# ml4ai/mliis

Hardware: AMD Instinct MI355X
Metric: inner-loop images/sec (EfficientLab-6-3, 224x224, 5-shot) (higher is better)
Workload: dtype f32 (the long-K decoder convs and their filter gradients with every operand split exactly into three bf16 terms on the matrix cores, 6 term products, f32 accumulate: fp32-equivalent products; everything else the fp32 instruction)

## Files before the change

### mliis_amd/csrc/conv_gemm_kernels.hpp

```cpp
#pragma once
#include <stdlib.h>

#include <type_traits>

#include "bn_fold.hpp"
#include "common.hpp"

namespace mliis {

typedef float f32x4 __attribute__((ext_vector_type(4)));

struct ConvGemmParams {
  const float* A;
  int lda;
  int Nimg, H, W;
  int C;
  int ntaps, dil, sign;
  const float* B;
  long long b_tap_stride;
  int ldb;
  int Nout;
  float* Cmat;
  int ldc;
  const float* bias;
// ... 826 lines not shown
            const float gq = (rok && cok) ? v * rscale : 0.f;
            const float xh = (side[r][j] - bmean[j]) * brstd[j];
            s1[j] += gq;
            s2[j] = fmaf(gq, xh, s2[j]);
          } else if constexpr (MODE == 1 || MODE == 2) {
            const float u0 = MODE == 2 ? swish_f(v) : v;
            const float u = rok ? u0 : 0.f;
            s1[j] += u;
            s2[j] = fmaf(u, u, s2[j]);
          }
        }
      }
    };
    if (bnb) epilogue(std::integral_constant<int, 3>{});
    else if (gated_part) epilogue(std::integral_constant<int, 4>{});
    else if (stats && p.stats_swish) epilogue(std::integral_constant<int, 2>{});
    else if (stats) epilogue(std::integral_constant<int, 1>{});
    else epilogue(std::integral_constant<int, 0>{});
    if (p.c_block != 0) {
      constexpr int QN = 4 * NT;
#pragma unroll
      for (int u = 0; u < NT; ++u) {
        const int e = lane + 64 * u;
        const int q4 = e >> 4, row = e & 15;
        const int m = rg * 16 + row, n = n0 + q4 * 4;
        const float4 v4 = ld4(&stage[wave][row * SROW + q4 * 4]);
        if (q4 < QN && m < M && n < p.Nout) {
          if (p.c_block == 4) {
            st4(p.Cmat + ((long long)(n >> 2) * M + m) * 4, v4);
          } else {
            float* d0 = p.Cmat + ((long long)(n >> 1) * M + m) * 2;
            *reinterpret_cast<float2*>(d0) = make_float2(v4.x, v4.y);
            *reinterpret_cast<float2*>(d0 + (long long)M * 2) = make_float2(v4.z, v4.w);
          }
        }
      }
    } else {
      constexpr int QN = 4 * NT;
#pragma unroll
      for (int u = 0; u < NT; ++u) {
        const int e = lane + 64 * u;
        const int row = e / QN, q4 = e - row * QN;
        const int m = rg * 16 + row, n = n0 + q4 * 4;
        const float4 v4 = ld4(&stage[wave][row * SROW + q4 * 4]);
        if (m < M && n < p.Nout) {
          if (PREC == 1 && p.out_bf16) stq(reinterpret_cast<bf16s*>(p.Cmat) + (long long)m * p.ldc + n, v4);
          else st4(p.Cmat + (long long)m * p.ldc + n, v4);
        }
      }
    }
    if (gated_part) {
#pragma unroll
      for (int j = 0; j < NT; ++j) {
        float a = gp0[j], b = gp1[j];
        a += __shfl_xor(a, 16, 64);
        b += __shfl_xor(b, 16, 64);
        a += __shfl_xor(a, 32, 64);
        b += __shfl_xor(b, 32, 64);
        const int n = n0 + j * 16 + l15;
        if (g == 0 && n < p.Nout) {
          p.gp_part[((long long)rg * 2 + 0) * p.Nout + n] = a;
          p.gp_part[((long long)rg * 2 + 1) * p.Nout + n] = b;
        }
      }
    }
    if constexpr (PF) {
#pragma unroll
      for (int kg = 0; kg < KC; ++kg) a_cur[kg] = a_nxt[kg];
      if constexpr (AIN) {
        if (rg + stride < row_groups) bn_in(rg + stride, a_cur, r_nxt, is_nxt);
      }
    } else {
      if (rg + stride < row_groups) {
        load_a(rg + stride, a_cur);
        load_side(rg + stride, r_cur, is_cur);
        bn_in(rg + stride, a_cur, r_cur, is_cur);
      }
    }
  }
  if (!stats) return;
#pragma unroll
  for (int j = 0; j < NT; ++j) {
    float a = s1[j], b = s2[j];
    a += __shfl_xor(a, 16, 64);
    b += __shfl_xor(b, 16, 64);
    a += __shfl_xor(a, 32, 64);
    b += __shfl_xor(b, 32, 64);
    if (g == 0) {
      red[wave][0][j * 16 + l15] = a;
      red[wave][1][j * 16 + l15] = b;
    }
  }
  __syncthreads();
  for (int idx = t; idx < 2 * 16 * NT; idx += 64 * kStreamWaves) {
    const int v = idx / (16 * NT), col = idx - v * (16 * NT);
    const int n = n0 + col;
    if (n < p.Nout) {
      float a = red[0][v][col];
#pragma unroll
      for (int wv = 1; wv < kStreamWaves; ++wv) a += red[wv][v][col];
      p.stats_part[((long long)blockIdx.x * 2 + v) * p.Nout + n] = a;
    }
  }
}

template <int KC, int NT, int WV, int PREC>
__global__ __launch_bounds__(64 * WV, (KC <= 6 && KC * NT <= 8) ? 4 : 2) void conv1x1_ksplit_k(ConvGemmParams p, int row_groups) {
  constexpr int BN = 16 * NT, RS = BN + 4, QN = BN / 4;
  __shared__ __attribute__((aligned(16))) float red[WV][16][RS];
  const int t = threadIdx.x, lane = t & 63, wave = t >> 6;
  const int l15 = lane & 15, g = lane >> 4;
  const int M = p.Nimg * p.H * p.W, HW = p.H * p.W;
  const int bx = blockIdx.x, by = blockIdx.y;
  const int n0 = by * BN;
  const int k0 = wave * 16 * KC;
  const __amdgpu_buffer_rsrc_t rA = __builtin_amdgcn_make_buffer_rsrc((void*)p.A, 0, kBufRecords, 0x00020000);
  const __amdgpu_buffer_rsrc_t rB = __builtin_amdgcn_make_buffer_rsrc((void*)p.B, 0, kBufRecords, 0x00020000);
  const __amdgpu_buffer_rsrc_t rS = __builtin_amdgcn_make_buffer_rsrc((void*)(p.a_scale ? p.a_scale : p.A), 0, kBufRecords, 0x00020000);
  const bool gated = p.a_scale != nullptr;
  float4 bv[KC][NT];
#pragma unroll
  for (int kg = 0; kg < KC; ++kg)
#pragma unroll
    for (int j = 0; j < NT; ++j) {
      const int n = n0 + j * 16 + l15, k = k0 + kg * 16 + g * 4;
      bv[kg][j] = buf_ld4(rB, (n < p.Nout && k < p.C) ? (unsigned)((n * p.ldb + k) * 4) : kOob);
    }
  constexpr int KC2 = (KC + 1) / 2;
  const float b_qscale = PREC == 2 ? fp8_weight_scale(p.b_amax) : 1.0f;
  const float out_scale = PREC == 2 ? 1.0f / (p.a_qscale * b_qscale) : 1.0f;
  bf16x8 bq16[PREC == 1 ? KC2 : 1][PREC == 1 ? NT : 1];
  long bq8[PREC == 2 ? KC2 : 1][PREC == 2 ? NT : 1];
  if constexpr (PREC != 0) {
#pragma unroll
    for (int k2 = 0; k2 < KC2; ++k2)
#pragma unroll
      for (int j = 0; j < NT; ++j) {
        const float4 lo = bv[2 * k2][j], hi = (2 * k2 + 1 < KC) ? bv[(2 * k2 + 1 < KC) ? 2 * k2 + 1 : 0][j] : f4zero();
        if constexpr (PREC == 1) bq16[k2][j] = pack_bf16x8(lo, hi);
        else bq8[k2][j] = pack_fp8x8(lo, hi, b_qscale);
      }
  }
  const bool fin = t < 16 * QN;
  const int frow = fin ? t / QN : 0, fq = fin ? t - frow * QN : 0;
  const int fn = n0 + fq * 4;
  const bool fcol = fin && fn < p.Nout;
  const float4 fbias = (fcol && p.bias != nullptr) ? ld4(p.bias + fn) : f4zero();
  float4 s1 = f4zero(), s2 = f4zero();
  const bool stats = p.stats_part != nullptr;
  const bool bnb = stats && p.bnb_x != nullptr;
  const float4 bmean = (bnb && fcol) ? ld4(p.bnb_mean + fn) : f4zero(), brstd = (bnb && fcol) ? ld4(p.bnb_rstd + fn) : f4zero();
  __shared__ __attribute__((aligned(16))) float sgate[2][16 * KC * WV];
  auto load_a = [&](int rg, float4* a) {
    const int m = rg * 16 + l15;
    const bool rok = rg < row_groups && m < M;
#pragma unroll
    for (int kg = 0; kg < KC; ++kg) {
      const int k = k0 + kg * 16 + g * 4;
      const bool ok = rok && k < p.C;
      if (PREC == 1 && p.a_bf16) a[kg] = buf_ld4_bf16(rA, ok ? (unsigned)((m * p.lda + k) * 2) : kOob);
      else a[kg] = buf_ld4(rA, ok ? (unsigned)((m * p.lda + k) * 4) : kOob);
    }
  };
  constexpr int GQ = 4 * KC * WV;
  auto gate_fetch = [&](int rg) {
    float4 v = f4zero();
    if (gated && t < 2 * GQ) {
      const int im = t / GQ, q = t - im * GQ;
      const int m0 = rg * 16;
      const int img = (m0 < M ? m0 : M - 1) / HW + im;
      if (rg < row_groups && img < p.Nimg && q * 4 < p.C) v = buf_ld4(rS, (unsigned)((img * p.C + q * 4) * 4));
    }
    return v;
  };
  auto gate_apply = [&](int rg, float4* a) {
    const int m = rg * 16 + l15;
    const int im = (m < M ? m : M - 1) / HW - (rg * 16 < M ? rg * 16 : M - 1) / HW;
#pragma unroll
    for (int kg = 0; kg < KC; ++kg) a[kg] = f4mul(a[kg], ld4(&sgate[im][k0 + kg * 16 + g * 4]));
  };
  int rg = bx;
  float4 a_cur[KC], a_nxt[KC];
  float4 gq = gate_fetch(rg);
  load_a(rg, a_cur);
  for (; rg < row_groups; rg += gridDim.x) {
    load_a(rg + gridDim.x, a_nxt);
    if (gated) {
      if (t < 2 * GQ) st4(&sgate[0][0] + t * 4, gq);
      __syncthreads();
      gate_apply(rg, a_cur);
      gq = gate_fetch(rg + gridDim.x);
    }
    float4 pre_dst = f4zero(), pre_x = f4zero();
    {
      const int mf = rg * 16 + frow;
      const bool pok = fcol && mf < M;
      if (p.accumulate && pok) pre_dst = ld4(p.Cmat + (long long)mf * p.ldc + fn);
      if (bnb && pok) pre_x = ld4(p.bnb_x + (long long)mf * p.bnb_ldx + fn);
    }
    f32x4 acc[NT];
#pragma unroll
    for (int j = 0; j < NT; ++j) acc[j] = (f32x4){0.f, 0.f, 0.f, 0.f};
    if constexpr (PREC == 0) {
#pragma unroll
      for (int kg = 0; kg < KC; ++kg)
#pragma unroll
        for (int sI = 0; sI < 4; ++sI) {
          const float a = sI == 0 ? a_cur[kg].x : sI == 1 ? a_cur[kg].y : sI == 2 ? a_cur[kg].z : a_cur[kg].w;
#pragma unroll
          for (int j = 0; j < NT; ++j) {
            const float b = sI == 0 ? bv[kg][j].x : sI == 1 ? bv[kg][j].y : sI == 2 ? bv[kg][j].z : bv[kg][j].w;
            acc[j] = __builtin_amdgcn_mfma_f32_16x16x4f32(a, b, acc[j], 0, 0, 0);
          }
        }
    } else {
#pragma unroll
      for (int k2 = 0; k2 < KC2; ++k2) {
        const float4 lo = a_cur[2 * k2], hi = (2 * k2 + 1 < KC) ? a_cur[(2 * k2 + 1 < KC) ? 2 * k2 + 1 : 0] : f4zero();
        if constexpr (PREC == 1) {
          const bf16x8 a8 = pack_bf16x8(lo, hi);
#pragma unroll
          for (int j = 0; j < NT; ++j) acc[j] = __builtin_amdgcn_mfma_f32_16x16x32_bf16(a8, bq16[k2][j], acc[j], 0, 0, 0);
        } else {
          const long a8 = pack_fp8x8(lo, hi, p.a_qscale);
#pragma unroll
          for (int j = 0; j < NT; ++j) acc[j] = __builtin_amdgcn_mfma_f32_16x16x32_fp8_fp8(a8, bq8[k2][j], acc[j], 0, 0, 0);
        }
      }
    }
#pragma unroll
    for (int r = 0; r < 4; ++r)
#pragma unroll
      for (int j = 0; j < NT; ++j) red[wave][g * 4 + r][j * 16 + l15] = PREC == 2 ? acc[j][r] * out_scale : acc[j][r];
    __syncthreads();
    const int m = rg * 16 + frow;
    if (fcol && m < M) {
      float4 v = ld4(&red[0][frow][fq * 4]);
#pragma unroll
      for (int w = 1; w < WV; ++w) v = f4add(v, ld4(&red[w][frow][fq * 4]));
      v = f4add(v, fbias);
      float* dst = p.Cmat + (long long)m * p.ldc + fn;
      if (p.accumulate) v = f4add(v, pre_dst);
      st4(dst, v);
      if (bnb) {
        const float4 xv = pre_x;
        if (p.bnb_scale != nullptr) v = f4scale(v, p.bnb_scale[m / HW]);
        const float4 xh = make_float4((xv.x - bmean.x) * brstd.x, (xv.y - bmean.y) * brstd.y, (xv.z - bmean.z) * brstd.z,
                                      (xv.w - bmean.w) * brstd.w);
        s1 = f4add(s1, v);
        s2 = f4fma(v, xh, s2);
      } else if (stats) {
        if (p.stats_swish) v = make_float4(swish_f(v.x), swish_f(v.y), swish_f(v.z), swish_f(v.w));
        s1 = f4add(s1, v);
        s2 = f4fma(v, v, s2);
      }
    }
    __syncthreads();
#pragma unroll
    for (int kg = 0; kg < KC; ++kg) a_cur[kg] = a_nxt[kg];
  }
  if (!stats) return;
  float4* fold = reinterpret_cast<float4*>(&red[0][0][0]);
  if (fin) {
    fold[(0 * 16 + frow) * QN + fq] = s1;
    fold[(1 * 16 + frow) * QN + fq] = s2;
  }
  __syncthreads();
  if (t < 2 * QN) {
    const int v = t / QN, q = t - v * QN;
    const int n = n0 + q * 4;
    if (n < p.Nout) {
      float4 a = fold[(v * 16) * QN + q];
#pragma unroll
      for (int r = 1; r < 16; ++r) a = f4add(a, fold[(v * 16 + r) * QN + q]);
      st4(p.stats_part + ((long long)bx * 2 + v) * p.Nout + n, a);
    }
  }
}

struct FilterGradParams {
  const float* X;
  int ldx;
  int Nimg, H, W;
  int C;
  int ntaps, dil;
  const float* dY;
  int lddy;
  int Nout;
  float* partial;
  int rows_per_split;
  const float* x_scale;
  int multitap;
  int x_bf16 = 0, dy_bf16 = 0;
};

template <int TMF, int NT>
struct FilterSm {
  static constexpr int BCI = 64 * TMF, BN = 16 * NT, BKM = 32;
  static constexpr int LDX = BCI + 16;
  static constexpr int LDD = (BN % 32 == 0) ? BN + 16 : BN;
  static constexpr int BUF_FLOATS = BKM * LDX + BKM * LDD;
};

template <int TMF, int NT, bool SC, bool BF>
__device__ __forceinline__ void conv_filter_grad2_body(const FilterGradParams& p, float* __restrict__ sm, int bx, int by, int bz) {
  constexpr int BCI = 64 * TMF, BN = 16 * NT, BKM = 32;
  constexpr int LDX = FilterSm<TMF, NT>::LDX;
  constexpr int LDD = FilterSm<TMF, NT>::LDD;
  constexpr int X_PER_THREAD = (BKM * (BCI / 4)) / 256;
  constexpr int D_TOTAL = BKM * (BN / 4);
  constexpr int D_PER_THREAD = (D_TOTAL + 255) / 256;
  constexpr int X_RSTEP = 256 / (BCI / 4);
  constexpr int BUF_FLOATS = FilterSm<TMF, NT>::BUF_FLOATS;
  constexpr int PF = (TMF == 2 && (SC || NT >= 8)) ? 1 : 2;

  const int t = threadIdx.x;
  const int lane = t & 63, wave = t >> 6;
  const int l15 = lane & 15, g = lane >> 4;
  const int M = p.Nimg * p.H * p.W;
  const bool mt = p.multitap != 0;
  const int cblocks = mt ? 1 : (p.C + BCI - 1) / BCI;
  const int tap = mt ? 0 : bx / cblocks;
  const int ci0 = mt ? 0 : (bx - tap * cblocks) * BCI;
  const int n0 = by * BN;
  const int mbeg = bz * p.rows_per_split;
  int mend = mbeg + p.rows_per_split;
  if (mend > M) mend = M;
  const int HW = p.H * p.W;
  const int adv_h = BKM / p.W, adv_w = BKM - adv_h * p.W;
  const bool xbf = BF && p.x_bf16 != 0, dbf = BF && p.dy_bf16 != 0;
  const int xb = xbf ? 2 : 4, db = dbf ? 2 : 4;

  const __amdgpu_buffer_rsrc_t rX = __builtin_amdgcn_make_buffer_rsrc((void*)p.X, 0, kBufRecords, 0x00020000);
  const __amdgpu_buffer_rsrc_t rD = __builtin_amdgcn_make_buffer_rsrc((void*)p.dY, 0, kBufRecords, 0x00020000);
  const __amdgpu_buffer_rsrc_t rS = __builtin_amdgcn_make_buffer_rsrc((void*)(SC ? p.x_scale : p.X), 0, kBufRecords, 0x00020000);

  const int x_cq = t % (BCI / 4);
  const int x_r0 = t / (BCI / 4);
  int l_tap = tap, l_c = ci0 + x_cq * 4;
  if (mt) {
    l_tap = (x_cq * 4) / p.C;
    l_c = x_cq * 4 - l_tap * p.C;
  }
  const bool x_cok = mt ? l_tap < p.ntaps : l_c < p.C;
  int dh = 0, dw = 0;
  if (p.ntaps > 1) {
    dh = (l_tap / 3 - 1) * p.dil;
    dw = (l_tap % 3 - 1) * p.dil;
  }
  int x_m[X_PER_THREAD], x_h[X_PER_THREAD], x_w[X_PER_THREAD], x_n[X_PER_THREAD];
  unsigned x_off[X_PER_THREAD];
#pragma unroll
  for (int i = 0; i < X_PER_THREAD; ++i) {
    const int m = mbeg + x_r0 + X_RSTEP * i;
    x_m[i] = m;
    x_n[i] = m / HW;
    const int rem = m - x_n[i] * HW;
    x_h[i] = rem / p.W;
    x_w[i] = rem - x_h[i] * p.W;
    x_off[i] = (unsigned)((((long long)m + (long long)dh * p.W + dw) * p.ldx + l_c) * xb);
  }
  const unsigned x_step = (unsigned)(BKM * p.ldx * xb);
  int d_m[D_PER_THREAD];
  unsigned d_off[D_PER_THREAD];
  bool d_ok[D_PER_THREAD];
#pragma unroll
  for (int i = 0; i < D_PER_THREAD; ++i) {
    const int idx = t + 256 * i;
    const int r = idx / (BN / 4), nq = idx - r * (BN / 4);
    d_m[i] = mbeg + r;
    d_ok[i] = (idx < D_TOTAL) && (n0 + nq * 4 < p.Nout);
    d_off[i] = (unsigned)((((long long)mbeg + r) * p.lddy + n0 + nq * 4) * db);
  }
  const unsigned d_step = (unsigned)(BKM * p.lddy * db);

  float4 rx[PF][X_PER_THREAD], rs[PF][X_PER_THREAD], rd[PF][D_PER_THREAD];
  auto load_chunk = [&](float4* rx_, float4* rs_, float4* rd_) {
#pragma unroll
    for (int i = 0; i < X_PER_THREAD; ++i) {
      const bool ok = x_cok & (x_m[i] < mend) & ((unsigned)(x_h[i] + dh) < (unsigned)p.H) & ((unsigned)(x_w[i] + dw) < (unsigned)p.W);
      if (BF && xbf) rx_[i] = buf_ld4_bf16(rX, ok ? x_off[i] : kOob);
      else rx_[i] = buf_ld4(rX, ok ? x_off[i] : kOob);
      if (SC) rs_[i] = buf_ld4(rS, ok ? (unsigned)((x_n[i] * p.C + l_c) * 4) : kOob);
      x_m[i] += BKM;
      x_off[i] += x_step;
      x_w[i] += adv_w;
      x_h[i] += adv_h;
      if (x_w[i] >= p.W) {
        x_w[i] -= p.W;
        ++x_h[i];
      }
      if (x_h[i] >= p.H) {
        const int k = x_h[i] / p.H;
        x_h[i] -= k * p.H;
        x_n[i] += k;
      }
    }
#pragma unroll
    for (int i = 0; i < D_PER_THREAD; ++i) {
      if (BF && dbf) rd_[i] = buf_ld4_bf16(rD, (d_ok[i] & (d_m[i] < mend)) ? d_off[i] : kOob);
      else rd_[i] = buf_ld4(rD, (d_ok[i] & (d_m[i] < mend)) ? d_off[i] : kOob);
      d_m[i] += BKM;
      d_off[i] += d_step;
    }
  };
  auto store_chunk = [&](float* buf, const float4* rx_, const float4* rs_, const float4* rd_) {
    float* smX = buf;
    float* smD = buf + BKM * LDX;
#pragma unroll
    for (int i = 0; i < X_PER_THREAD; ++i) {
      float4 v = rx_[i];
      if (SC) v = f4mul(v, rs_[i]);
      st4(smX + (x_r0 + X_RSTEP * i) * LDX + x_cq * 4, v);
    }
#pragma unroll
    for (int i = 0; i < D_PER_THREAD; ++i) {
      const int idx = t + 256 * i;
      if (idx < D_TOTAL) {
        const int r = idx / (BN / 4), nq = idx - r * (BN / 4);
        st4(smD + r * LDD + nq * 4, rd_[i]);
      }
    }
  };

  f32x4 acc[TMF][NT];
#pragma unroll
  for (int i = 0; i < TMF; ++i)
#pragma unroll
    for (int j = 0; j < NT; ++j) acc[i][j] = (f32x4){0.f, 0.f, 0.f, 0.f};

  load_chunk(rx[0], rs[0], rd[0]);
  store_chunk(sm, rx[0], rs[0], rd[0]);
  if (PF == 2) load_chunk(rx[PF - 1], rs[PF - 1], rd[PF - 1]);
  __syncthreads();
  int cur = 0;
  const bool wave_live = mt ? wave * TMF * 16 < p.ntaps * p.C : ci0 + wave * TMF * 16 < p.C;
  auto step = [&](auto UC) {
    constexpr int U = decltype(UC)::value;
    constexpr int NX = (U + 1) % PF;
    load_chunk(rx[U], rs[U], rd[U]);
    const float* smX = sm + cur * BUF_FLOATS;
    const float* smD = smX + BKM * LDX;
    if (!wave_live) {
    } else if constexpr (BF) {
      bf16x8 a8[TMF], b8[NT];
#pragma unroll
      for (int kk = 0; kk < BKM / 4; ++kk) {
        const int mrow = kk * 4 + g;
#pragma unroll
        for (int i = 0; i < TMF; ++i) a8[i][kk] = (__bf16)smX[mrow * LDX + (wave * TMF + i) * 16 + l15];
#pragma unroll
        for (int j = 0; j < NT; ++j) b8[j][kk] = (__bf16)smD[mrow * LDD + j * 16 + l15];
      }
#pragma unroll
      for (int i = 0; i < TMF; ++i)
#pragma unroll
        for (int j = 0; j < NT; ++j) acc[i][j] = __builtin_amdgcn_mfma_f32_16x16x32_bf16(a8[i], b8[j], acc[i][j], 0, 0, 0);
    } else
#pragma unroll
    for (int kk = 0; kk < BKM / 4; ++kk) {
      const int mrow = kk * 4 + g;
      float a[TMF], b[NT];
#pragma unroll
      for (int i = 0; i < TMF; ++i) a[i] = smX[mrow * LDX + (wave * TMF + i) * 16 + l15];
#pragma unroll
      for (int j = 0; j < NT; ++j) b[j] = smD[mrow * LDD + j * 16 + l15];
#pragma unroll
      for (int i = 0; i < TMF; ++i)
#pragma unroll
        for (int j = 0; j < NT; ++j) acc[i][j] = __builtin_amdgcn_mfma_f32_16x16x4f32(a[i], b[j], acc[i][j], 0, 0, 0);
    }
    store_chunk(sm + (cur ^ 1) * BUF_FLOATS, rx[NX], rs[NX], rd[NX]);
    cur ^= 1;
    __syncthreads();
  };
  typedef std::integral_constant<int, 0> U0;
  typedef std::integral_constant<int, 1 % PF> U1;
  const int nchunks = (mend - mbeg + BKM - 1) / BKM;
  int it = 0;
  for (; it + 4 <= nchunks; it += 4) {
    step(U0{});
    step(U1{});
    step(U0{});
    step(U1{});
  }
  if (it < nchunks) step(U0{});
  if (it + 1 < nchunks) step(U1{});
  if (it + 2 < nchunks) step(U0{});

  const long long Ktot = (long long)p.ntaps * p.C;
#pragma unroll
  for (int i = 0; i < TMF; ++i)
#pragma unroll
    for (int r = 0; r < 4; ++r) {
      const int ci = ci0 + (wave * TMF + i) * 16 + g * 4 + r;
      if (ci >= (mt ? p.ntaps * p.C : p.C)) continue;
#pragma unroll
      for (int j = 0; j < NT; ++j) {
        const int n = n0 + j * 16 + l15;
        if (n < p.Nout) p.partial[((long long)bz * Ktot + (long long)tap * p.C + ci) * p.Nout + n] = acc[i][j][r];
      }
    }
}

template <int TMF, int NT, bool SC, bool BF>
__global__ __launch_bounds__(256, 2) void conv_filter_grad2_k(FilterGradParams p) {
  __shared__ __attribute__((aligned(16))) float sm[2 * FilterSm<TMF, NT>::BUF_FLOATS];
  conv_filter_grad2_body<TMF, NT, SC, BF>(p, sm, blockIdx.x, blockIdx.y, blockIdx.z);
}

constexpr int kFilterDescWords = 16;
template <int TMF, int NT, bool SC, bool BF>
__global__ __launch_bounds__(256, 2) void conv_filter_grad2_batched_k(const long long* __restrict__ desc, int nprob) {
  __shared__ __attribute__((aligned(16))) float sm[2 * FilterSm<TMF, NT>::BUF_FLOATS];
  const int b = blockIdx.x;
  int j = 0;
  for (int k = 1; k < nprob; ++k)
    if (b >= (int)desc[k * kFilterDescWords + 15]) j = k;
  const long long* d = desc + (long long)j * kFilterDescWords;
  const int ks = (int)(d[11] & 0xff);
  const FilterGradParams p{reinterpret_cast<const float*>(d[0]), (int)d[4], (int)d[6], (int)d[7], (int)d[8], (int)d[9], ks * ks, (int)d[12],
                           reinterpret_cast<const float*>(d[1]), (int)d[5], (int)d[10], reinterpret_cast<float*>(d[3]),
                           (int)(d[13] & 0xffffffffLL), reinterpret_cast<const float*>(d[2]), (int)(d[13] >> 32),
                           (int)((d[11] >> 8) & 1), (int)((d[11] >> 9) & 1)};
  const int gx = (int)(d[14] & 0xfffff), gy = (int)((d[14] >> 20) & 0xfffff);
  const int local = b - (int)d[15];
  const int bx = local % gx, r = local / gx;
  conv_filter_grad2_body<TMF, NT, SC, BF>(p, sm, bx, r % gy, r / gy);
}

struct GemmPlan {
  int tm, nt, gx, gy, gz, chunks_per_split;
  int sk_full, sk_rem, sk_parts, sk_ipp, sk_nchunks, sk_smax;
  size_t sk_slab_floats() const { return sk_parts > 0 ? (size_t)sk_rem * sk_smax * 64 * (16 * nt) : 0; }
};

static inline bool gemm_narrow(int ntaps, int C) { return ntaps > 1 && C < 32; }

template <int PREC>
static void launch_gemm_sk_t(const GemmPlan& g, const ConvGemmParams& p, float* slab, hipStream_t stream) {
  const SkPlan k{g.sk_full, g.sk_rem, g.sk_parts, g.sk_ipp, g.sk_nchunks, g.sk_smax, g.gy, slab};
  dim3 grid(g.sk_full + g.sk_parts), block(256);
  constexpr int PF = 2;
#define SKL(NT_)                                                                                       \
  hipLaunchKernelGGL((conv_gemm_sk_k<NT_, PF, false, PREC>), grid, block, 0, stream, p, k);           \
  hipLaunchKernelGGL((sk_fixup_k<NT_>), dim3(g.sk_rem), dim3(1024), 0, stream, p, k);                  \
  break;
  switch (g.nt) {
    case 1: SKL(1)
    case 2: SKL(2)
    case 3: SKL(3)
    case 4: SKL(4)
    case 5: SKL(5)
    case 6: SKL(6)
    case 7: SKL(7)
    default: SKL(8)
  }
#undef SKL
}

template <int PREC>
static void launch_gemm_t(const GemmPlan& g, const ConvGemmParams& p, hipStream_t stream) {
  dim3 grid(g.gx, g.gy, g.gz), block(256);
  const bool sp = p.partial != nullptr, sc = p.a_scale != nullptr, narrow = gemm_narrow(p.ntaps, p.C);
#define NK(TM_, NT_, SC_, SP_) hipLaunchKernelGGL((conv_gemm_nk_k<TM_, NT_, (TM_ == 1 ? 2 : 1), SC_, SP_, false, PREC>), grid, block, 0, stream, p)
#define L(TM_, NT_)                                  \
  if (TM_ == 1 && narrow) {                          \
    hipLaunchKernelGGL((conv_gemm_nk_k<1, NT_, 2, false, false, true, PREC>), grid, block, 0, stream, p); \
  } else if (TM_ == 1 && sp) {                       \
    if (sc) NK(1, NT_, true, true);                  \
    else NK(1, NT_, false, true);                    \
  } else if (sc) NK(TM_, NT_, true, false);          \
  else NK(TM_, NT_, false, false);                   \
  break;
#define ROW(TM_)       \
  switch (g.nt) {      \
    case 1: L(TM_, 1)  \
    case 2: L(TM_, 2)  \
    case 3: L(TM_, 3)  \
    case 4: L(TM_, 4)  \
    case 5: L(TM_, 5)  \
    case 6: L(TM_, 6)  \
    case 7: L(TM_, 7)  \
    default: L(TM_, 8) \
  }
  if (g.tm == 2) {
    ROW(2)
  } else {
    ROW(1)
  }
#undef ROW
#undef L
#undef NK
}

#define MLIIS_STREAM_INSTANCES(X)                                                                                            \
  X(1, 1, 1) X(1, 2, 1) X(1, 3, 1) X(1, 4, 1) X(1, 5, 0) X(1, 6, 0) X(1, 7, 0) X(1, 8, 0) X(2, 1, 1) X(2, 2, 1) X(2, 3, 1) \
  X(2, 4, 1) X(3, 1, 1) X(3, 2, 1) X(4, 1, 1) X(4, 2, 1) X(5, 1, 1) X(6, 1, 1) X(7, 1, 1)
#define MLIIS_KSPLIT_INSTANCES(X)                                                                                  \
  X(1, 1) X(1, 2) X(1, 3) X(1, 4) X(1, 5) X(1, 6) X(1, 7) X(2, 1) X(2, 2) X(2, 3) X(2, 4) X(3, 1) X(3, 2) X(4, 1) \
  X(4, 2) X(4, 3) X(5, 1) X(5, 2) X(6, 1) X(6, 2) X(7, 1)

static inline bool stream_instance(int kc, int nt, bool ain) {
#define X(KC_, NT_, AIN_) if (kc == KC_ && nt == NT_) return !ain || AIN_;
  MLIIS_STREAM_INSTANCES(X)
#undef X
  return false;
}
static inline bool ksplit_instance(int kc, int nt) {
#define X(KC_, NT_) if (kc == KC_ && nt == NT_) return true;
  MLIIS_KSPLIT_INSTANCES(X)
#undef X
  return false;
}

template <int PREC, bool AIN>
static bool launch_stream_t(int kc, int nt, dim3 grid, const ConvGemmParams& p, int row_groups, hipStream_t stream) {
  dim3 block(64 * kStreamWaves);
#define X(KC_, NT_, AIN_)                                                                                               \
  if constexpr (!AIN || AIN_)                                                                                           \
    if (kc == KC_ && nt == NT_) {                                                                                       \
      hipLaunchKernelGGL((conv1x1_stream_k<KC_, NT_, PREC, AIN>), grid, block, 0, stream, p, row_groups);              \
      return true;                                                                                                      \
    }
  MLIIS_STREAM_INSTANCES(X)
#undef X
  return false;
}
template <int PREC>
static bool launch_ksplit_t(int kc, int nt, dim3 grid, const ConvGemmParams& p, int row_groups, hipStream_t stream) {
  dim3 block(512);
#define X(KC_, NT_)                                                                                        \
  if (kc == KC_ && nt == NT_) {                                                                            \
    hipLaunchKernelGGL((conv1x1_ksplit_k<KC_, NT_, 8, PREC>), grid, block, 0, stream, p, row_groups);     \
    return true;                                                                                           \
  }
  MLIIS_KSPLIT_INSTANCES(X)
#undef X
  return false;
}

struct FilterPlan {
  int tmf, nt, gx, gy, gz, rows_per_split, multitap;
};

template <bool BF>
static bool launch_filter_batched_t(int tmf, int nt, bool sc, const long long* desc, int nprob, int blocks, hipStream_t stream) {
  dim3 grid(blocks), block(256);
#define L(T_, NT_)                                                                                                            \
  if (sc) hipLaunchKernelGGL((conv_filter_grad2_batched_k<T_, NT_, true, BF>), grid, block, 0, stream, desc, nprob);          \
  else hipLaunchKernelGGL((conv_filter_grad2_batched_k<T_, NT_, false, BF>), grid, block, 0, stream, desc, nprob);            \
  break;
#define ROW(T_)       \
  switch (nt) {       \
    case 1: L(T_, 1)  \
    case 2: L(T_, 2)  \
    case 3: L(T_, 3)  \
    case 4: L(T_, 4)  \
    case 5: L(T_, 5)  \
    case 6: L(T_, 6)  \
    case 7: L(T_, 7)  \
    case 8: L(T_, 8)  \
    default: return false; \
  }
  if (tmf == 2) {
    ROW(2)
  } else if (tmf == 1) {
    ROW(1)
  } else {
    return false;
  }
#undef ROW
#undef L
  return true;
}

template <bool BF>
static void launch_filter_t(const FilterPlan& f, const FilterGradParams& p, hipStream_t stream) {
  dim3 grid(f.gx, f.gy, f.gz), block(256);
#define L(T_, NT_)                                                                                                   \
  if (p.x_scale) hipLaunchKernelGGL((conv_filter_grad2_k<T_, NT_, true, BF>), grid, block, 0, stream, p);           \
  else hipLaunchKernelGGL((conv_filter_grad2_k<T_, NT_, false, BF>), grid, block, 0, stream, p);                         \
  break;
#define ROW(T_)       \
  switch (f.nt) {     \
    case 1: L(T_, 1)  \
    case 2: L(T_, 2)  \
    case 3: L(T_, 3)  \
    case 4: L(T_, 4)  \
    case 5: L(T_, 5)  \
    case 6: L(T_, 6)  \
    case 7: L(T_, 7)  \
    default: L(T_, 8) \
  }
  if (f.tmf == 2) {
    ROW(2)
  } else {
    ROW(1)
  }
#undef ROW
#undef L
}

constexpr int kX3Block = 3072;
constexpr int kX3DescWords = 8;
__device__ __forceinline__ void x3_pack_block(const float* __restrict__ theta, char* __restrict__ images, const long long* __restrict__ desc,
                                              int ndesc, int b, int t) {
  int j = 0;
  for (int k = 1; k < ndesc; ++k)
    if (b >= (int)(desc[k * kX3DescWords + 6] >> 8)) j = k;
  const long long* d = desc + (long long)j * kX3DescWords;
  const float* w = theta + d[0];
  const int taps = (int)d[1], cin_total = (int)d[2], cout = (int)d[3], ci_begin = (int)d[4], cin = (int)d[5], mode = (int)(d[6] & 0xff);
  const int local = b - (int)(d[6] >> 8);
  const int nn = mode == 0 ? cout : cin, kc = mode == 0 ? cin : cout;
  const int ncol16 = (nn + 15) / 16;
  const int chunk = local / ncol16, c16 = local - chunk * ncol16;
  const int nl = t & 15, kq = t >> 4;
  const int n = c16 * 16 + nl;
  const int k = chunk * 32 + kq * 4;
  const int tap = k / kc, c = k - tap * kc;
  float4 v = f4zero();
  if (n < nn && tap < taps) {
    if (mode == 0) {
      const float* s = w + ((long long)tap * cin_total + ci_begin + c) * cout + n;
      v = make_float4(s[0], s[cout], s[2 * (long long)cout], s[3 * (long long)cout]);
    } else {
      v = ld4(w + ((long long)tap * cin_total + ci_begin + n) * cout + c);
    }
  }
  uint2 h, m, l;
  split3(v, h, m, l);
  char* dst = images + d[7] + (long long)local * kX3Block + (kq & 3) * 256 + nl * 16 + (kq >> 2) * 8;
  *reinterpret_cast<uint2*>(dst) = h;
  *reinterpret_cast<uint2*>(dst + 1024) = m;
  *reinterpret_cast<uint2*>(dst + 2048) = l;
}


void launch_gemm_bf16(const GemmPlan& g, const ConvGemmParams& p, hipStream_t stream);
void launch_gemm_sk_bf16(const GemmPlan& g, const ConvGemmParams& p, float* slab, hipStream_t stream);
void launch_gemm_fp8(const GemmPlan& g, const ConvGemmParams& p, hipStream_t stream);
bool launch_stream_lowp(int precision, int kc, int nt, dim3 grid, const ConvGemmParams& p, int row_groups, hipStream_t stream, bool ain = false);
bool launch_ksplit_lowp(int precision, int kc, int nt, dim3 grid, const ConvGemmParams& p, int row_groups, hipStream_t stream);
void launch_filter_bf16(const FilterPlan& f, const FilterGradParams& p, hipStream_t stream);
bool launch_filter_batched_bf16(int tmf, int nt, bool sc, const long long* desc, int nprob, int blocks, hipStream_t stream);
bool launch_filter_batched_x3(int nt, const long long* desc, int nprob, int blocks, int tile_ci, hipStream_t stream);

}
```

Baseline: 3583.

## Balance filter-gradient MFMA tiles across waves for partially filled blocks

For the fp32 filter-gradient kernel, each block now counts the live 16x16 output tiles (ci by n) and spreads them evenly over the four waves as row or column segments. Previously each wave owned a fixed band of TMF ci-tiles across all NT n-tiles, so small C or Nout left waves idle or doing masked work. This should balance MFMA work within a block for narrow layers. It costs a runtime switch over segment shapes, more template instantiations and register pressure, and a separate store path.

Result: no change. 3598 (median of 5 runs) (+0.4%).

```diff
diff --git a/mliis_amd/csrc/conv_gemm_kernels.hpp b/mliis_amd/csrc/conv_gemm_kernels.hpp
--- a/mliis_amd/csrc/conv_gemm_kernels.hpp
+++ b/mliis_amd/csrc/conv_gemm_kernels.hpp
@@ -1152,6 +1152,15 @@
   static constexpr int BUF_FLOATS = BKM * LDX + BKM * LDD;
 };
 
+constexpr bool filter_pairs_ok(int tmf, int nt) {
+  for (int ni = 1; ni <= 4 * tmf; ++ni)
+    for (int nj = 1; nj <= nt; ++nj) {
+      const int per = (ni * nj + 3) / 4;
+      if (ni * ((nj + per - 1) / per) > 4 && nj * ((ni + per - 1) / per) > 4) return false;
+    }
+  return true;
+}
+
 template <int TMF, int NT, bool SC, bool BF>
 __device__ __forceinline__ void conv_filter_grad2_body(const FilterGradParams& p, float* __restrict__ sm, int bx, int by, int bz) {
   constexpr int BCI = 64 * TMF, BN = 16 * NT, BKM = 32;
@@ -1273,11 +1282,34 @@
     }
   };
 
-  f32x4 acc[TMF][NT];
-#pragma unroll
-  for (int i = 0; i < TMF; ++i)
-#pragma unroll
-    for (int j = 0; j < NT; ++j) acc[i][j] = (f32x4){0.f, 0.f, 0.f, 0.f};
+  constexpr int S = TMF * NT;
+  constexpr bool PAIRS = !BF && filter_pairs_ok(TMF, NT);
+  f32x4 acc[S];
+#pragma unroll
+  for (int s = 0; s < S; ++s) acc[s] = (f32x4){0.f, 0.f, 0.f, 0.f};
+  int nw = 0, pa = 0, pb = 0;
+  bool seg_col = false;
+  if constexpr (PAIRS) {
+    const int wv = __builtin_amdgcn_readfirstlane(wave);
+    const int crem = mt ? p.ntaps * p.C : p.C - ci0, nrem = p.Nout - n0;
+    int ni = (crem + 15) >> 4, nj = (nrem + 15) >> 4;
+    ni = ni > 4 * TMF ? 4 * TMF : (ni < 1 ? 1 : ni);
+    nj = nj > NT ? NT : (nj < 1 ? 1 : nj);
+    const int per = (ni * nj + 3) >> 2;
+    const int row_pieces = (nj + per - 1) / per, col_pieces = (ni + per - 1) / per;
+    if (ni * row_pieces <= 4) {
+      const int i = wv / row_pieces, j = (wv - i * row_pieces) * per;
+      nw = i < ni ? (nj - j < per ? nj - j : per) : 0;
+      pa = i * 16;
+      pb = j * 16;
+    } else {
+      const int j = wv / col_pieces, i = (wv - j * col_pieces) * per;
+      nw = j < nj ? (ni - i < per ? ni - i : per) : 0;
+      pa = i * 16;
+      pb = j * 16;
+      seg_col = nw > 1;
+    }
+  }
 
   load_chunk(rx[0], rs[0], rd[0]);
   store_chunk(sm, rx[0], rs[0], rd[0]);
@@ -1285,12 +1317,44 @@
   __syncthreads();
   int cur = 0;
   const bool wave_live = mt ? wave * TMF * 16 < p.ntaps * p.C : ci0 + wave * TMF * 16 < p.C;
+  auto mma_seg = [&](auto COLC, auto NSC, const float* smX, const float* smD) {
+    constexpr bool COL = decltype(COLC)::value;
+    constexpr int NS = decltype(NSC)::value;
+    if constexpr (NS <= S) {
+      constexpr int NA = COL ? NS : 1, NB = COL ? 1 : NS;
+#pragma unroll
+      for (int kk = 0; kk < BKM / 4; ++kk) {
+        const int mrow = kk * 4 + g;
+        float a[NA], b[NB];
+#pragma unroll
+        for (int s = 0; s < NA; ++s) a[s] = smX[mrow * LDX + pa + s * 16 + l15];
+#pragma unroll
+        for (int s = 0; s < NB; ++s) b[s] = smD[mrow * LDD + pb + s * 16 + l15];
+#pragma unroll
+        for (int s = 0; s < NS; ++s) acc[s] = __builtin_amdgcn_mfma_f32_16x16x4f32(a[COL ? s : 0], b[COL ? 0 : s], acc[s], 0, 0, 0);
+      }
+    }
+  };
   auto step = [&](auto UC) {
     constexpr int U = decltype(UC)::value;
     constexpr int NX = (U + 1) % PF;
     load_chunk(rx[U], rs[U], rd[U]);
     const float* smX = sm + cur * BUF_FLOATS;
     const float* smD = smX + BKM * LDX;
+    if constexpr (PAIRS) {
+      typedef std::false_type Row;
+      typedef std::true_type Col;
+      switch (seg_col ? nw + 4 : nw) {
+        case 1: mma_seg(Row{}, std::integral_constant<int, 1>{}, smX, smD); break;
+        case 2: mma_seg(Row{}, std::integral_constant<int, 2>{}, smX, smD); break;
+        case 3: mma_seg(Row{}, std::integral_constant<int, 3>{}, smX, smD); break;
+        case 4: mma_seg(Row{}, std::integral_constant<int, 4>{}, smX, smD); break;
+        case 6: mma_seg(Col{}, std::integral_constant<int, 2>{}, smX, smD); break;
+        case 7: mma_seg(Col{}, std::integral_constant<int, 3>{}, smX, smD); break;
+        case 8: mma_seg(Col{}, std::integral_constant<int, 4>{}, smX, smD); break;
+        default: break;
+      }
+    } else
     if (!wave_live) {
     } else if constexpr (BF) {
       bf16x8 a8[TMF], b8[NT];
@@ -1305,7 +1369,7 @@
 #pragma unroll
       for (int i = 0; i < TMF; ++i)
 #pragma unroll
-        for (int j = 0; j < NT; ++j) acc[i][j] = __builtin_amdgcn_mfma_f32_16x16x32_bf16(a8[i], b8[j], acc[i][j], 0, 0, 0);
+        for (int j = 0; j < NT; ++j) acc[i * NT + j] = __builtin_amdgcn_mfma_f32_16x16x32_bf16(a8[i], b8[j], acc[i * NT + j], 0, 0, 0);
     } else
 #pragma unroll
     for (int kk = 0; kk < BKM / 4; ++kk) {
@@ -1318,7 +1382,7 @@
 #pragma unroll
       for (int i = 0; i < TMF; ++i)
 #pragma unroll
-        for (int j = 0; j < NT; ++j) acc[i][j] = __builtin_amdgcn_mfma_f32_16x16x4f32(a[i], b[j], acc[i][j], 0, 0, 0);
+        for (int j = 0; j < NT; ++j) acc[i * NT + j] = __builtin_amdgcn_mfma_f32_16x16x4f32(a[i], b[j], acc[i * NT + j], 0, 0, 0);
     }
     store_chunk(sm + (cur ^ 1) * BUF_FLOATS, rx[NX], rs[NX], rd[NX]);
     cur ^= 1;
@@ -1339,16 +1403,31 @@
   if (it + 2 < nchunks) step(U0{});
 
   const long long Ktot = (long long)p.ntaps * p.C;
+  const int climit = mt ? p.ntaps * p.C : p.C;
+  if constexpr (PAIRS) {
+#pragma unroll
+    for (int s = 0; s < S; ++s) {
+      if (s >= nw) break;
+      const int cb = ci0 + pa + (seg_col ? s * 16 : 0), nb = n0 + pb + (seg_col ? 0 : s * 16);
+#pragma unroll
+      for (int r = 0; r < 4; ++r) {
+        const int ci = cb + g * 4 + r;
+        const int n = nb + l15;
+        if (ci < climit && n < p.Nout) p.partial[((long long)bz * Ktot + (long long)tap * p.C + ci) * p.Nout + n] = acc[s][r];
+      }
+    }
+    return;
+  }
 #pragma unroll
   for (int i = 0; i < TMF; ++i)
 #pragma unroll
     for (int r = 0; r < 4; ++r) {
       const int ci = ci0 + (wave * TMF + i) * 16 + g * 4 + r;
-      if (ci >= (mt ? p.ntaps * p.C : p.C)) continue;
+      if (ci >= climit) continue;
 #pragma unroll
       for (int j = 0; j < NT; ++j) {
         const int n = n0 + j * 16 + l15;
-        if (n < p.Nout) p.partial[((long long)bz * Ktot + (long long)tap * p.C + ci) * p.Nout + n] = acc[i][j][r];
+        if (n < p.Nout) p.partial[((long long)bz * Ktot + (long long)tap * p.C + ci) * p.Nout + n] = acc[i * NT + j][r];
       }
     }
 }
```
